# lean-dojo/ReProver

Hardware: NVIDIA H100
Metric: premises encoded/sec (reindex_corpus, ByT5-small, seq_len<=512) (higher is better)
Workload: dtype bf16

## Files before the change

reprover_b200/csrc/rpx_attention.cu:

```cuda
#include "rpx_common.cuh"
#include "rpx_kernels.cuh"
#include "rpx_ptx.cuh"

namespace rpx {

namespace {

constexpr int kHD = 64;
constexpr int kQT = 64;
constexpr int kKT = 64;
constexpr int kAttnThreads = 160;
constexpr int kTileBytes = 64 * 128;

constexpr int kOffQ = 0;
constexpr int kOffK = kTileBytes;
constexpr int kOffV = 3 * kTileBytes;
constexpr int kOffBias = 5 * kTileBytes;

__host__ __device__ constexpr int bias_floats(int R) { return ((2 * R + 1) + 3) & ~3; }
size_t attention_smem_bytes(int R) { return 1024 + kOffBias + (size_t)bias_floats(R) * 4 + 64; }

RPX_DEVICE float fast_exp2(float x) {
  float y;
  asm("ex2.approx.ftz.f32 %0, %1;" : "=f"(y) : "f"(x));
  return y;
}

__global__ void __launch_bounds__(kAttnThreads, 2)
t5_attention_kernel(const __grid_constant__ CUtensorMap tm_q, const __grid_constant__ CUtensorMap tm_kv,
                    __nv_bfloat16* __restrict__ out, const int32_t* __restrict__ cu_seqlens,
                    const float* __restrict__ bias_lut, int n_heads, int R, int ld_out) {
  const int seq = blockIdx.z, head = blockIdx.y, qt = blockIdx.x;
  pdl_launch_dependents();
  const int t0 = cu_seqlens[seq];
  const int len = cu_seqlens[seq + 1] - t0;
  const int q0 = qt * kQT;
  if (q0 >= len) return;

  extern __shared__ uint8_t smem_raw[];
  const uint32_t raw = smem_u32(smem_raw);
  uint8_t* smem = smem_raw + ((1024 - (raw & 1023)) & 1023);
  float* sBias = reinterpret_cast<float*>(smem + kOffBias);
  const int lut_w = 2 * R + 1;
  uint64_t* bars = reinterpret_cast<uint64_t*>(smem + kOffBias + bias_floats(R) * 4);
  uint64_t* bar_q = bars + 0;
  uint64_t* bar_k = bars + 1;
  uint64_t* bar_v = bars + 3;
  uint64_t* bar_free = bars + 5;

  const int warp = threadIdx.x >> 5, lane = threadIdx.x & 31;
  const int inner = n_heads * kHD;
  const int n_kt = (len + kKT - 1) / kKT;

  for (int i = threadIdx.x; i < lut_w; i += kAttnThreads) sBias[i] = bias_lut[head * lut_w + i];
  if (warp == 4) {
    if (elect_one()) {
      mbar_init(bar_q, 1);
      for (int b = 0; b < 2; ++b) {
        mbar_init(&bar_k[b], 1);
        mbar_init(&bar_v[b], 1);
        mbar_init(&bar_free[b], 128);
      }
      fence_mbar_init();
    }
    __syncwarp();
  }
  __syncthreads();

  if (warp == 4) {
    if (elect_one()) {
      const int kcol = inner + head * kHD, vcol = 2 * inner + head * kHD;
      pdl_wait();
      mbar_arrive_expect_tx(bar_q, kTileBytes);
      tma_load_2d(smem + kOffQ, &tm_q, bar_q, head * kHD, t0 + q0);
      for (int kt = 0; kt < n_kt; ++kt) {
        const int b = kt & 1;
        if (kt >= 2) mbar_wait<0>(&bar_free[b], ((kt >> 1) - 1) & 1);
        mbar_arrive_expect_tx(&bar_k[b], kTileBytes);
        tma_load_2d(smem + kOffK + b * kTileBytes, &tm_kv, &bar_k[b], kcol, t0 + kt * kKT);
        mbar_arrive_expect_tx(&bar_v[b], kTileBytes);
        tma_load_2d(smem + kOffV + b * kTileBytes, &tm_kv, &bar_v[b], vcol, t0 + kt * kKT);
      }
    }
  } else {
    const int g = lane >> 2, cq = 2 * (lane & 3);
    const int qpos0 = q0 + warp * 16 + g, qpos1 = qpos0 + 8;
    const float kLog2e = 1.4426950408889634f;
    float m0 = -INFINITY, m1 = -INFINITY, l0 = 0.f, l1 = 0.f;
    float o[32];
#pragma unroll
    for (int i = 0; i < 32; ++i) o[i] = 0.f;
    const uint64_t q_desc = make_smem_desc_kmajor_sw128(smem_u32(smem + kOffQ));
    mbar_wait<0>(bar_q, 0);
    for (int kt = 0; kt < n_kt; ++kt) {
      const int b = kt & 1;
      const uint32_t ph = (kt >> 1) & 1;
      const int kb = kt * kKT;
      float sc[32];
      mbar_wait<0>(&bar_k[b], ph);
      {
        const uint64_t k_desc = make_smem_desc_kmajor_sw128(smem_u32(smem + kOffK + b * kTileBytes));
        wgmma_fence_operand(sc);
        wgmma_fence();
#pragma unroll
        for (int k = 0; k < kHD / 16; ++k) wgmma_m64n64k16_ss(sc, q_desc + 2 * k, k_desc + 2 * k, k != 0);
        wgmma_commit();
        wgmma_wait<0>();
        wgmma_fence_operand(sc);
      }
      float mx0 = -INFINITY, mx1 = -INFINITY;
#pragma unroll
      for (int j = 0; j < 8; ++j) {
#pragma unroll
        for (int e = 0; e < 2; ++e) {
          const int key = kb + 8 * j + cq + e;
          const bool ok = key < len;
          const float b0 = sBias[min(max(key - qpos0 + R, 0), 2 * R)];
          const float b1 = sBias[min(max(key - qpos1 + R, 0), 2 * R)];
          sc[4 * j + e] = ok ? sc[4 * j + e] + b0 : -INFINITY;
          sc[4 * j + 2 + e] = ok ? sc[4 * j + 2 + e] + b1 : -INFINITY;
          mx0 = fmaxf(mx0, sc[4 * j + e]);
          mx1 = fmaxf(mx1, sc[4 * j + 2 + e]);
        }
      }
      mx0 = fmaxf(mx0, __shfl_xor_sync(0xffffffffu, mx0, 1));
      mx0 = fmaxf(mx0, __shfl_xor_sync(0xffffffffu, mx0, 2));
      mx1 = fmaxf(mx1, __shfl_xor_sync(0xffffffffu, mx1, 1));
      mx1 = fmaxf(mx1, __shfl_xor_sync(0xffffffffu, mx1, 2));
      const float mn0 = fmaxf(m0, mx0), mn1 = fmaxf(m1, mx1);
      const float scale0 = fast_exp2((m0 - mn0) * kLog2e), scale1 = fast_exp2((m1 - mn1) * kLog2e);
      m0 = mn0;
      m1 = mn1;
      const float mb0 = mn0 * kLog2e, mb1 = mn1 * kLog2e;
      uint32_t pa[4][4];
      float ls0 = 0.f, ls1 = 0.f;
#pragma unroll
      for (int j = 0; j < 8; ++j) {
        const float p00 = fast_exp2(fmaf(sc[4 * j], kLog2e, -mb0));
        const float p01 = fast_exp2(fmaf(sc[4 * j + 1], kLog2e, -mb0));
        const float p10 = fast_exp2(fmaf(sc[4 * j + 2], kLog2e, -mb1));
        const float p11 = fast_exp2(fmaf(sc[4 * j + 3], kLog2e, -mb1));
        ls0 += p00 + p01;
        ls1 += p10 + p11;
        pa[j >> 1][(j & 1) * 2] = pack_bf16x2(p00, p01);
        pa[j >> 1][(j & 1) * 2 + 1] = pack_bf16x2(p10, p11);
      }
      l0 = l0 * scale0 + ls0;
      l1 = l1 * scale1 + ls1;
#pragma unroll
      for (int j = 0; j < 8; ++j) {
        o[4 * j] *= scale0;
        o[4 * j + 1] *= scale0;
        o[4 * j + 2] *= scale1;
        o[4 * j + 3] *= scale1;
      }
      mbar_wait<0>(&bar_v[b], ph);
      {
        const uint32_t v_base = smem_u32(smem + kOffV + b * kTileBytes);
        wgmma_fence_operand(o);
        wgmma_fence();
#pragma unroll
        for (int c = 0; c < kKT / 16; ++c)
          wgmma_m64n64k16_rs_bmn(o, pa[c], make_smem_desc_mnmajor_sw128(v_base + c * 2048), 1);
        wgmma_commit();
        wgmma_wait<0>();
        wgmma_fence_operand(o);
      }
      mbar_arrive(&bar_free[b]);
    }
    l0 += __shfl_xor_sync(0xffffffffu, l0, 1);
    l0 += __shfl_xor_sync(0xffffffffu, l0, 2);
    l1 += __shfl_xor_sync(0xffffffffu, l1, 1);
    l1 += __shfl_xor_sync(0xffffffffu, l1, 2);
    const float inv0 = 1.f / l0, inv1 = 1.f / l1;
    __nv_bfloat16* dst0 = out + (int64_t)(t0 + qpos0) * ld_out + head * kHD + cq;
    __nv_bfloat16* dst1 = out + (int64_t)(t0 + qpos1) * ld_out + head * kHD + cq;
#pragma unroll
    for (int j = 0; j < 8; ++j) {
      if (qpos0 < len) *reinterpret_cast<uint32_t*>(dst0 + 8 * j) = pack_bf16x2(o[4 * j] * inv0, o[4 * j + 1] * inv0);
      if (qpos1 < len) *reinterpret_cast<uint32_t*>(dst1 + 8 * j) = pack_bf16x2(o[4 * j + 2] * inv1, o[4 * j + 3] * inv1);
    }
  }
}

}

int launch_t5_attention(const __nv_bfloat16* qkv, __nv_bfloat16* out, const int32_t* cu_seqlens,
                        const float* bias_lut, int n_tokens, int n_seqs, int max_len, int n_heads, int d_kv,
                        int max_distance, cudaStream_t stream) {
  RPX_REQUIRE(d_kv == kHD, RPX_ERR_UNSUPPORTED, "attention: d_kv=%d (only 64 is implemented)", d_kv);
  RPX_REQUIRE(n_seqs > 0 && max_len > 0 && n_tokens > 0, RPX_ERR_INVALID, "attention: empty batch");
  RPX_REQUIRE(n_seqs <= 65535 && n_heads <= 65535, RPX_ERR_UNSUPPORTED, "attention: grid limits exceeded");
  const int inner = n_heads * d_kv;
  DeviceInfo dev;
  RPX_TRY(get_device_info(&dev));
  CUtensorMap tm_q, tm_kv;
  RPX_TRY(make_tmap_bf16_2d(&tm_kv, qkv, (uint64_t)n_tokens, (uint64_t)3 * inner, (uint64_t)3 * inner, kKT));
  RPX_TRY(make_tmap_bf16_2d(&tm_q, qkv, (uint64_t)n_tokens, (uint64_t)3 * inner, (uint64_t)3 * inner, kQT));
  const size_t smem = attention_smem_bytes(max_distance);
  RPX_REQUIRE(smem <= 100 * 1024, RPX_ERR_UNSUPPORTED, "attention: bias table too large (%zu B of shared memory)", smem);
  static thread_local int configured = -1;
// ... 12 lines not shown
```

reprover_b200/csrc/rpx_encoder.cu:

```cuda
#include <math.h>

#include <new>
#include <vector>

#include "rpx_gemm_launch.cuh"
#include "rpx_kernels.cuh"

namespace rpx {

namespace {

constexpr int kBlockN = 128;

struct LayerW {
  const __nv_bfloat16* qkv;
  const __nv_bfloat16* o;
  const __nv_bfloat16* wi;
  const __nv_bfloat16* wo;
};

struct ProfRec {
  int cls;
  cudaEvent_t a, b;
};

}

}

extern "C" int32_t rpx_t5_relative_bucket(int32_t relative_position, int32_t num_buckets, int32_t max_distance) {
  int nb = num_buckets / 2;
  int ret = relative_position > 0 ? nb : 0;
  int n = relative_position < 0 ? -relative_position : relative_position;
  const int max_exact = nb / 2;
  if (n < max_exact) return ret + n;
  float v = logf((float)n / (float)max_exact) / (float)log((double)max_distance / (double)max_exact) *
            (float)(nb - max_exact);
  int large = max_exact + (int)v;
  if (large > nb - 1) large = nb - 1;
  return ret + large;
}

struct rpx_encoder {
  rpx_t5_config cfg;
  int inner = 0;
// ... 144 lines not shown
  }
  ~Prof() {
    if (!e->profiling) return;
    cudaEventRecord(b, st);
    e->prof_pending.push_back({cls, a, b});
  }
  cudaEvent_t get() {
    if (!e->event_pool.empty()) {
      cudaEvent_t ev = e->event_pool.back();
      e->event_pool.pop_back();
      return ev;
    }
    cudaEvent_t ev;
    cudaEventCreate(&ev);
    return ev;
  }
};

constexpr int kLatBlockN = 64;
constexpr int kLatStages = 6;
constexpr int kLatSmallM = 64;
constexpr int kLatSmallStages = 12;
constexpr int kLatSmallMMaxTokens = 384;
constexpr int kPdlMaxTokens = 16384;

struct PdlScope {
  explicit PdlScope(bool on) { set_pdl_scope(on); }
  ~PdlScope() { set_pdl_scope(false); }
};

int ss_parts(int d_model, bool latency) { return ceil_div(d_model, latency ? 32 : 128); }


int qkv_gemm(bool latency, int T, const void* A, const void* B, int N, int K, const RowScale& rs, __nv_bfloat16* out,
             const void* prefetch, size_t prefetch_bytes, cudaStream_t st) {
  EpiStoreBF16::Params ep{out, N, rs};
  if (!latency) return launch_gemm<kBlockN, EpiStoreBF16>(A, K, B, K, T, N, K, ep, st);
  if (T <= kLatSmallMMaxTokens)
    return launch_gemm<kLatBlockN, EpiStoreBF16, false, kLatSmallStages, false, kLatSmallM>(A, K, B, K, T, N, K, ep, st, 0,
                                                                                             prefetch, prefetch_bytes);
  return launch_gemm<kLatBlockN, EpiStoreBF16, false, kLatStages>(A, K, B, K, T, N, K, ep, st, 0, prefetch, prefetch_bytes);
}

template <int RES_BUFS, int STAGES, int CLUSTER>
int residual_gemm(bool latency, int T, const void* A, const void* B, int N, int K, float* h32, __nv_bfloat16* h16,
                  float* ss_out, cudaStream_t st) {
  EpiResidualParams ep{h32, h16, N, ss_out, T};
  if (!latency) return launch_gemm_ws<EpiWsResidual<RES_BUFS>, STAGES, CLUSTER>(A, K, B, K, T, N, K, ep, st);
  if (T <= kLatSmallMMaxTokens)
    return launch_gemm<kLatBlockN, EpiResidualChunkSS, false, kLatSmallStages, false, kLatSmallM>(A, K, B, K, T, N, K, ep, st);
  return launch_gemm<kLatBlockN, EpiResidualChunkSS, false, kLatStages>(A, K, B, K, T, N, K, ep, st);
}
int oproj_gemm(bool latency, int T, const void* A, const void* B, int N, int K, float* h32, __nv_bfloat16* h16,
               float* ss_out, cudaStream_t st) {
  return residual_gemm<2, 4, 1>(latency, T, A, B, N, K, h32, h16, ss_out, st);
}
int ffn_down_gemm(bool latency, int T, const void* A, const void* B, int N, int K, float* h32, __nv_bfloat16* h16,
                  float* ss_out, cudaStream_t st) {
  return residual_gemm<5, 3, 2>(latency, T, A, B, N, K, h32, h16, ss_out, st);
}

int ffn_up_gemm(bool latency, int T, const void* A, const void* B, int N, int K, const RowScale& rs,
                __nv_bfloat16* out, cudaStream_t st) {
  RPX_REQUIRE(N % 256 == 0, RPX_ERR_UNSUPPORTED, "ffn-up gemm: N=%d must be a multiple of 256 (2 x d_ff, d_ff %% 128 == 0)", N);
  const int F = N / 2;
  if (!latency) {
    EpiWsGeGLU::Params ep{out, F, rs};
    return launch_gemm_ws<EpiWsGeGLU, kFfnUpStages, kFfnUpCluster>(A, K, B, K, T, N, K, ep, st);
  }
  if (T <= kBlockM) {
// ... 405 lines not shown
```

reprover_b200/csrc/rpx_gemm_launch.cuh:

```cuda
#pragma once
#include "rpx_common.cuh"
#include "rpx_gemm.cuh"
#include "rpx_gemm_ws.cuh"

namespace rpx {

constexpr int kGemmStages = 4;

template <int BLOCK_N, class Epi, bool M_FASTEST = false, int STAGES = kGemmStages, bool SPLIT_B = false, int BM = kBlockM>
int launch_gemm(const void* A, int64_t lda, const void* B, int64_t ldb, int M, int N, int K,
                const typename Epi::Params& ep, cudaStream_t stream, int grid_limit = 0, const void* prefetch_ptr = nullptr,
                size_t prefetch_bytes = 0) {
  using Cfg = GemmCfg<BLOCK_N, STAGES, BM>;
  static_assert(BM == kBlockM || (!M_FASTEST && Epi::kWarps == 4), "64-row tiles: encoder epilogues with one warp per lane group");
  RPX_REQUIRE(M > 0 && N > 0 && K > 0, RPX_ERR_INVALID, "gemm: empty problem M=%d N=%d K=%d", M, N, K);
  RPX_REQUIRE(K % kBlockK == 0, RPX_ERR_UNSUPPORTED, "gemm: K=%d must be a multiple of %d", K, kBlockK);
  RPX_REQUIRE(M_FASTEST || N % 32 == 0, RPX_ERR_UNSUPPORTED, "gemm: N=%d must be a multiple of 32", N);
  DeviceInfo dev;
  RPX_TRY(get_device_info(&dev));
  CUtensorMap tmA, tmB;
  RPX_TRY(make_tmap_bf16_2d(&tmA, A, (uint64_t)M, (uint64_t)K, (uint64_t)lda, BM));
  RPX_TRY(make_tmap_bf16_2d(&tmB, B, (uint64_t)N, (uint64_t)K, (uint64_t)ldb, SPLIT_B ? BLOCK_N / 2 : BLOCK_N));
  RPX_REQUIRE(!SPLIT_B || N % BLOCK_N == 0, RPX_ERR_UNSUPPORTED, "gemm: split-B tiles need N %% %d == 0", BLOCK_N);
  const int tiles_m = ceil_div(M, BM);
  const int tiles_n = ceil_div(N, BLOCK_N);
  const size_t smem = Cfg::smem_bytes(Epi::kSmemBytes);
  RPX_REQUIRE(smem <= dev.smem_optin, RPX_ERR_UNSUPPORTED, "gemm: needs %zu B smem, device allows %zu",
              smem, dev.smem_optin);
  auto kern = gemm_tc_kernel<BLOCK_N, STAGES, Epi, M_FASTEST, SPLIT_B, BM>;
  static thread_local int configured_dev = -1;
  if (configured_dev != dev.device) {
    RPX_CUDA_OK(cudaFuncSetAttribute(kern, cudaFuncAttributeMaxDynamicSharedMemorySize, (int)smem));
    configured_dev = dev.device;
  }
  int grid = tiles_m * tiles_n;
  int cap = grid_limit > 0 ? grid_limit : dev.num_sms;
  if (grid > cap) grid = cap;
  L2Prefetch pf{prefetch_ptr, (uint32_t)prefetch_bytes, grid, next_timeline_slot()};
  if (prefetch_ptr != nullptr && prefetch_bytes > 0 && prefetch_bytes < ((size_t)1 << 32) && grid < dev.num_sms)
    grid = dev.num_sms;
  RPX_CUDA_OK(launch_pdl(kern, dim3(grid), dim3(gemm_threads<Epi>()), smem, stream, pdl_enabled(), tmA, tmB, M, N, K, tiles_m,
                         tiles_n, 1, ep, pf));
  return RPX_OK;
}

constexpr int kFfnUpStages = 4;
constexpr int kFfnUpCluster = 2;

template <class Epi, int STAGES, int CLUSTER>
int launch_gemm_ws(const void* A, int64_t lda, const void* B, int64_t ldb, int M, int N, int K,
                   const typename Epi::Params& ep, cudaStream_t stream) {
  RPX_REQUIRE(M > 0 && N > 0 && K > 0, RPX_ERR_INVALID, "gemm: empty problem M=%d N=%d K=%d", M, N, K);
  RPX_REQUIRE(K % kBlockK == 0, RPX_ERR_UNSUPPORTED, "gemm: K=%d must be a multiple of %d", K, kBlockK);
  RPX_REQUIRE(N % 32 == 0, RPX_ERR_UNSUPPORTED, "gemm: N=%d must be a multiple of 32", N);
  DeviceInfo dev;
  RPX_TRY(get_device_info(&dev));
  CUtensorMap tmA, tmB, tmR;
  RPX_TRY(make_tmap_bf16_2d(&tmA, A, (uint64_t)M, (uint64_t)K, (uint64_t)lda, kBlockM));
  RPX_TRY(make_tmap_bf16_2d(&tmB, B, (uint64_t)N, (uint64_t)K, (uint64_t)ldb, kWsBlockN / CLUSTER));
  if constexpr (Epi::kResBufs > 0)
    RPX_TRY(make_tmap_2d(&tmR, 4, ep.h32, (uint64_t)M, (uint64_t)N, (uint64_t)ep.ld, kResChunkCols, 64, 128));
  else
    tmR = tmA;
  const int tiles_m = ceil_div(M, kBlockM);
  const int tiles_n = ceil_div(N, kWsBlockN);
  const size_t smem = WsCfg<STAGES, Epi::kResBufs>::kSmemBytes;
  RPX_REQUIRE(smem <= dev.smem_optin, RPX_ERR_UNSUPPORTED, "gemm: needs %zu B smem, device allows %zu", smem,
              dev.smem_optin);
  auto kern = gemm_ws_kernel<Epi, STAGES, CLUSTER>;
  static thread_local int configured_dev = -1;
  static thread_local int max_clusters = 0;
  if (configured_dev != dev.device) {
    RPX_CUDA_OK(cudaFuncSetAttribute(kern, cudaFuncAttributeMaxDynamicSharedMemorySize, (int)smem));
    cudaLaunchConfig_t cfg{};
    cfg.gridDim = dim3(CLUSTER * dev.num_sms);
    cfg.blockDim = dim3(kWsThreads);
    cfg.dynamicSmemBytes = smem;
    cudaLaunchAttribute at[1];
    at[0].id = cudaLaunchAttributeClusterDimension;
    at[0].val.clusterDim.x = CLUSTER;
    at[0].val.clusterDim.y = 1;
    at[0].val.clusterDim.z = 1;
    cfg.attrs = at;
    cfg.numAttrs = 1;
    RPX_CUDA_OK(cudaOccupancyMaxActiveClusters(&max_clusters, kern, &cfg));
    RPX_REQUIRE(max_clusters > 0, RPX_ERR_UNSUPPORTED, "gemm: no cluster of %d CTAs with %zu B smem fits the device",
                CLUSTER, smem);
    configured_dev = dev.device;
  }
  int clusters = ceil_div(tiles_m, CLUSTER) * tiles_n;
  if (clusters > max_clusters) clusters = max_clusters;
  RPX_CUDA_OK(launch_pdl<CLUSTER>(kern, dim3(CLUSTER * clusters), dim3(kWsThreads), smem, stream, pdl_enabled(), tmA,
                                  tmB, tmR, M, N, K, tiles_m, tiles_n, ep));
  return RPX_OK;
}

template <class Epi, int STAGES = kGemmStages>
int launch_gemm_pair(const void* A, int64_t lda, const void* B, int64_t ldb, int M, int N, int K,
                     const typename Epi::Params& ep, cudaStream_t stream) {
  constexpr int BLOCK_N = 128;
  using Cfg = GemmCfg<BLOCK_N, STAGES, kBlockM>;
  RPX_REQUIRE(M > 0 && N > 0 && K > 0, RPX_ERR_INVALID, "gemm: empty problem M=%d N=%d K=%d", M, N, K);
// ... 39 lines not shown
```

reprover_b200/csrc/rpx_gemm_ws.cuh:

```cuda
#pragma once
#include "rpx_gemm.cuh"

namespace rpx {

constexpr int kWsBlockN = 256;
constexpr int kWsThreads = 384;
constexpr int kResChunkCols = 32;
constexpr int kResChunkBytes = 64 * kResChunkCols * 4;

template <int STAGES, int RES_BUFS>
struct WsCfg {
  static_assert(2 * STAGES + 4 * RES_BUFS <= 32, "barrier block holds 32 mbarriers");
  static constexpr int kABytes = kBlockM * kBlockK * 2;
  static constexpr int kBBytes = kWsBlockN * kBlockK * 2;
  static constexpr int kStageBytes = kABytes + kBBytes;
  static constexpr int kRingBytes = STAGES * kStageBytes;
  static constexpr int kResBytes = 2 * RES_BUFS * kResChunkBytes;
  static constexpr size_t kSmemBytes = (size_t)kRingBytes + kResBytes + 1024 + 256;
};

struct FragCtx {
  int m0, n0;
  int n_blk;
  int n_cols;
  int M, N;
  int r0;
  int q;
};

struct ResStream {
  float* buf;
  uint64_t* full;
  uint64_t* empty;
};

template <class Epi, int STAGES, int CLUSTER>
__global__ void __launch_bounds__(kWsThreads, 1)
gemm_ws_kernel(const __grid_constant__ CUtensorMap tmA, const __grid_constant__ CUtensorMap tmB,
               const __grid_constant__ CUtensorMap tmR, int M, int N, int K, int tiles_m, int tiles_n,
               typename Epi::Params ep) {
  static_assert(CLUSTER == 1 || CLUSTER == 2, "one CTA, or a pair sharing the B tile");
  using Cfg = WsCfg<STAGES, Epi::kResBufs>;
  constexpr int R = Epi::kResBufs;
  extern __shared__ uint8_t smem_raw[];
  const uint32_t raw_addr = smem_u32(smem_raw);
  uint8_t* smem = smem_raw + ((1024 - (raw_addr & 1023)) & 1023);
  uint8_t* sA = smem;
  uint8_t* sB = smem + STAGES * Cfg::kABytes;
  float* sR = reinterpret_cast<float*>(smem + Cfg::kRingBytes);
  uint64_t* full = reinterpret_cast<uint64_t*>(smem + Cfg::kRingBytes + Cfg::kResBytes);
  uint64_t* empty = full + STAGES;
  uint64_t* rfull = empty + STAGES;
  uint64_t* rempty = rfull + 2 * R;

  const int warp = threadIdx.x >> 5;
  const int wg = warp >> 2;
  const int num_kb = K / kBlockK;
  const int rank = CLUSTER > 1 ? (int)cluster_ctarank() : 0;
  const int num_units = (tiles_m + CLUSTER - 1) / CLUSTER * tiles_n;
  const int u0 = (int)blockIdx.x / CLUSTER;
  const int u_step = (int)gridDim.x / CLUSTER;
  auto unit_m = [&](int u) { return CLUSTER * (u / tiles_n) + rank; };

  if (threadIdx.x == 0) {
    tma_prefetch_desc(&tmA);
    tma_prefetch_desc(&tmB);
    if (R > 0) tma_prefetch_desc(&tmR);
    for (int s = 0; s < STAGES; ++s) {
      mbar_init(&full[s], 1);
      mbar_init(&empty[s], CLUSTER * 8);
    }
    for (int s = 0; s < 2 * R; ++s) {
      mbar_init(&rfull[s], 1);
      mbar_init(&rempty[s], 128);
    }
    fence_mbar_init();
  }
  __syncthreads();
  if (CLUSTER > 1) cluster_sync_all();
  pdl_launch_dependents();
  pdl_wait();

  if (wg == 0) {
    setmaxnreg_dec<40>();
    if (warp == 0 && elect_one()) {
      int stage = 0;
      uint32_t phase = 0;
      for (int u = u0; u < num_units; u += u_step) {
        const int m_blk = unit_m(u), n_blk = u % tiles_n;
        for (int kb = 0; kb < num_kb; ++kb) {
          mbar_wait(&empty[stage], phase ^ 1);
          mbar_arrive_expect_tx(&full[stage], Cfg::kStageBytes);
          tma_load_2d(sA + stage * Cfg::kABytes, &tmA, &full[stage], kb * kBlockK, m_blk * kBlockM);
          if constexpr (CLUSTER == 1) {
            tma_load_2d(sB + stage * Cfg::kBBytes, &tmB, &full[stage], kb * kBlockK, n_blk * kWsBlockN);
          } else {
            constexpr int H = kWsBlockN / 2;
            tma_load_2d_multicast(sB + stage * Cfg::kBBytes + rank * H * kBlockK * 2, &tmB, &full[stage], kb * kBlockK,
                                  n_blk * kWsBlockN + rank * H, (uint16_t)0x3);
          }
          if (++stage == STAGES) {
            stage = 0;
            phase ^= 1;
          }
        }
      }
    } else if (R > 0 && (warp == 1 || warp == 2) && elect_one()) {
      const int w = warp - 1;
      float* buf = sR + w * R * (kResChunkBytes / 4);
      uint64_t* rf = rfull + w * R;
      uint64_t* re = rempty + w * R;
      int b = 0;
      uint32_t phase = 0;
      for (int u = u0; u < num_units; u += u_step) {
        const int row0 = unit_m(u) * kBlockM + 64 * w;
        const int n0 = (u % tiles_n) * kWsBlockN;
        const int n_cols = N - n0 < kWsBlockN ? N - n0 : kWsBlockN;
        if (row0 >= M) continue;
        for (int col = 0; col < n_cols; col += kResChunkCols) {
          mbar_wait(&re[b], phase ^ 1);
          mbar_arrive_expect_tx(&rf[b], kResChunkBytes);
          tma_load_2d(buf + b * (kResChunkBytes / 4), &tmR, &rf[b], n0 + col, row0);
          if (++b == R) {
            b = 0;
            phase ^= 1;
          }
        }
      }
    }
  } else {
    setmaxnreg_inc<232>();
    const int cw = wg - 1;
    const int lane = threadIdx.x & 31;
    Epi epi(ep, ResStream{sR + cw * R * (kResChunkBytes / 4), rfull + cw * R, rempty + cw * R});
    float acc[128];
    int stage = 0;
    uint32_t phase = 0;
    auto release = [&](int st) {
      __syncwarp();
      if (lane == 0) {
        mbar_arrive(&empty[st]);
        if (CLUSTER > 1) mbar_arrive_cluster(&empty[st], (uint32_t)(rank ^ 1));
      }
    };
    for (int u = u0; u < num_units; u += u_step) {
      FragCtx c;
      c.n_blk = u % tiles_n;
      c.m0 = unit_m(u) * kBlockM;
      c.n0 = c.n_blk * kWsBlockN;
      c.n_cols = N - c.n0 < kWsBlockN ? N - c.n0 : kWsBlockN;
      c.M = M;
      c.N = N;
      c.r0 = c.m0 + 64 * cw + 16 * (warp & 3) + (lane >> 2);
      c.q = lane & 3;
      int prev = 0;
      for (int kb = 0; kb < num_kb; ++kb) {
        mbar_wait(&full[stage], phase);
        const uint64_t a_desc = make_smem_desc_kmajor_sw128(smem_u32(sA + stage * Cfg::kABytes)) + 512 * cw;
        const uint64_t b_desc = make_smem_desc_kmajor_sw128(smem_u32(sB + stage * Cfg::kBBytes));
        wgmma_fence_operand(acc);
        wgmma_fence();
#pragma unroll
        for (int k = 0; k < kBlockK / kMmaK; ++k) wgmma_m64n256k16_ss(acc, a_desc + 2 * k, b_desc + 2 * k, (kb | k) != 0);
        wgmma_commit();
        if (kb == 0) epi.prefetch(c);
        if (kb > 0) {
          wgmma_wait<1>();
          release(prev);
        }
        prev = stage;
        if (++stage == STAGES) {
          stage = 0;
          phase ^= 1;
        }
      }
      wgmma_wait<0>();
      wgmma_fence_operand(acc);
      release(prev);
      epi.tile(c, acc);
    }
  }
  if (CLUSTER > 1) {
    __syncwarp();
    cluster_sync_all();
  }
}


struct EpiWsStoreF32 {
  using Params = EpiStoreF32::Params;
  static constexpr int kResBufs = 0;
  Params p;
  __device__ EpiWsStoreF32(const Params& p_, const ResStream&) : p(p_) {}
  __device__ void prefetch(const FragCtx&) {}
  __device__ void tile(const FragCtx& c, const float (&acc)[128]) {
#pragma unroll
    for (int j = 0; j < 32; ++j) {
      if (8 * j < c.n_cols) {
        float* dst = p.C + (size_t)c.r0 * p.ldc + c.n0 + 8 * j + 2 * c.q;
        if (c.r0 < c.M) *reinterpret_cast<float2*>(dst) = make_float2(acc[4 * j], acc[4 * j + 1]);
        if (c.r0 + 8 < c.M) *reinterpret_cast<float2*>(dst + 8 * (size_t)p.ldc) = make_float2(acc[4 * j + 2], acc[4 * j + 3]);
      }
    }
  }
};

struct EpiWsGeGLU {
  struct Params {
    __nv_bfloat16* out;
    int ldo;
    RowScale rs;
  };
  static constexpr int kResBufs = 0;
  Params p;
  float rs0 = 0.f, rs1 = 0.f;
  __device__ EpiWsGeGLU(const Params& p_, const ResStream&) : p(p_) {}
  __device__ void prefetch(const FragCtx& c) {
    rs0 = c.r0 < c.M ? p.rs.get(c.r0) : 0.f;
    rs1 = c.r0 + 8 < c.M ? p.rs.get(c.r0 + 8) : 0.f;
  }
// ... 93 lines not shown
```

reprover_b200/csrc/rpx_ptx.cuh:

```cuda
#pragma once
#include <cuda_runtime.h>
#include <cuda_bf16.h>
#include <stdint.h>

namespace rpx {

#define RPX_DEVICE __device__ __forceinline__

RPX_DEVICE uint32_t smem_u32(const void* p) {
  return static_cast<uint32_t>(__cvta_generic_to_shared(p));
}

RPX_DEVICE uint32_t lane_id() { return threadIdx.x & 31; }

RPX_DEVICE uint32_t elect_one() {
  uint32_t pred = 0;
  asm volatile(
      "{\n"
      ".reg .b32 rx;\n"
      ".reg .pred px;\n"
      "elect.sync rx|px, 0xFFFFFFFF;\n"
      "@px mov.s32 %0, 1;\n"
      "}\n"
      : "+r"(pred));
// ... 135 lines not shown
RPX_DEVICE void wgmma_wait() {
  asm volatile("wgmma.wait_group.sync.aligned %0;" ::"n"(N) : "memory");
}
template <int R>
RPX_DEVICE void wgmma_fence_operand(float (&d)[R]) {
#pragma unroll
  for (int i = 0; i < R; ++i) asm volatile("" : "+f"(d[i])::"memory");
}

RPX_DEVICE void wgmma_m64n64k16_ss(float (&d)[32], uint64_t desc_a, uint64_t desc_b, uint32_t accumulate) {
  asm volatile(
      "{\n"
      ".reg .pred p;\n"
      "setp.ne.b32 p, %34, 0;\n"
      "wgmma.mma_async.sync.aligned.m64n64k16.f32.bf16.bf16 "
      "{%0, %1, %2, %3, %4, %5, %6, %7, %8, %9, %10, %11, %12, %13, %14, %15, %16, %17, %18, %19, %20, %21, %22, %23, %24, %25, %26, %27, %28, %29, %30, %31}, %32, %33, p, 1, 1, 0, 0;\n"
      "}\n"
      : "+f"(d[0]), "+f"(d[1]), "+f"(d[2]), "+f"(d[3]), "+f"(d[4]), "+f"(d[5]), "+f"(d[6]), "+f"(d[7]), "+f"(d[8]), "+f"(d[9]), "+f"(d[10]), "+f"(d[11]), "+f"(d[12]), "+f"(d[13]), "+f"(d[14]), "+f"(d[15]), "+f"(d[16]), "+f"(d[17]), "+f"(d[18]), "+f"(d[19]), "+f"(d[20]), "+f"(d[21]), "+f"(d[22]), "+f"(d[23]), "+f"(d[24]), "+f"(d[25]), "+f"(d[26]), "+f"(d[27]), "+f"(d[28]), "+f"(d[29]), "+f"(d[30]), "+f"(d[31])
      : "l"(desc_a), "l"(desc_b), "r"(accumulate));
}

RPX_DEVICE void wgmma_m64n128k16_ss(float (&d)[64], uint64_t desc_a, uint64_t desc_b, uint32_t accumulate) {
  asm volatile(
      "{\n"
      ".reg .pred p;\n"
      "setp.ne.b32 p, %66, 0;\n"
      "wgmma.mma_async.sync.aligned.m64n128k16.f32.bf16.bf16 "
      "{%0, %1, %2, %3, %4, %5, %6, %7, %8, %9, %10, %11, %12, %13, %14, %15, %16, %17, %18, %19, %20, %21, %22, %23, %24, %25, %26, %27, %28, %29, %30, %31, %32, %33, %34, %35, %36, %37, %38, %39, %40, %41, %42, %43, %44, %45, %46, %47, %48, %49, %50, %51, %52, %53, %54, %55, %56, %57, %58, %59, %60, %61, %62, %63}, %64, %65, p, 1, 1, 0, 0;\n"
      "}\n"
      : "+f"(d[0]), "+f"(d[1]), "+f"(d[2]), "+f"(d[3]), "+f"(d[4]), "+f"(d[5]), "+f"(d[6]), "+f"(d[7]), "+f"(d[8]), "+f"(d[9]), "+f"(d[10]), "+f"(d[11]), "+f"(d[12]), "+f"(d[13]), "+f"(d[14]), "+f"(d[15]), "+f"(d[16]), "+f"(d[17]), "+f"(d[18]), "+f"(d[19]), "+f"(d[20]), "+f"(d[21]), "+f"(d[22]), "+f"(d[23]), "+f"(d[24]), "+f"(d[25]), "+f"(d[26]), "+f"(d[27]), "+f"(d[28]), "+f"(d[29]), "+f"(d[30]), "+f"(d[31]), "+f"(d[32]), "+f"(d[33]), "+f"(d[34]), "+f"(d[35]), "+f"(d[36]), "+f"(d[37]), "+f"(d[38]), "+f"(d[39]), "+f"(d[40]), "+f"(d[41]), "+f"(d[42]), "+f"(d[43]), "+f"(d[44]), "+f"(d[45]), "+f"(d[46]), "+f"(d[47]), "+f"(d[48]), "+f"(d[49]), "+f"(d[50]), "+f"(d[51]), "+f"(d[52]), "+f"(d[53]), "+f"(d[54]), "+f"(d[55]), "+f"(d[56]), "+f"(d[57]), "+f"(d[58]), "+f"(d[59]), "+f"(d[60]), "+f"(d[61]), "+f"(d[62]), "+f"(d[63])
      : "l"(desc_a), "l"(desc_b), "r"(accumulate));
}

RPX_DEVICE void wgmma_m64n256k16_ss(float (&d)[128], uint64_t desc_a, uint64_t desc_b, uint32_t accumulate) {
  asm volatile(
      "{\n"
      ".reg .pred p;\n"
      "setp.ne.b32 p, %130, 0;\n"
      "wgmma.mma_async.sync.aligned.m64n256k16.f32.bf16.bf16 "
      "{%0, %1, %2, %3, %4, %5, %6, %7, %8, %9, %10, %11, %12, %13, %14, %15, %16, %17, %18, %19, %20, %21, %22, %23, %24, %25, %26, %27, %28, %29, %30, %31, %32, %33, %34, %35, %36, %37, %38, %39, %40, %41, %42, %43, %44, %45, %46, %47, %48, %49, %50, %51, %52, %53, %54, %55, %56, %57, %58, %59, %60, %61, %62, %63, %64, %65, %66, %67, %68, %69, %70, %71, %72, %73, %74, %75, %76, %77, %78, %79, %80, %81, %82, %83, %84, %85, %86, %87, %88, %89, %90, %91, %92, %93, %94, %95, %96, %97, %98, %99, %100, %101, %102, %103, %104, %105, %106, %107, %108, %109, %110, %111, %112, %113, %114, %115, %116, %117, %118, %119, %120, %121, %122, %123, %124, %125, %126, %127}, %128, %129, p, 1, 1, 0, 0;\n"
      "}\n"
      : "+f"(d[0]), "+f"(d[1]), "+f"(d[2]), "+f"(d[3]), "+f"(d[4]), "+f"(d[5]), "+f"(d[6]), "+f"(d[7]), "+f"(d[8]), "+f"(d[9]), "+f"(d[10]), "+f"(d[11]), "+f"(d[12]), "+f"(d[13]), "+f"(d[14]), "+f"(d[15]), "+f"(d[16]), "+f"(d[17]), "+f"(d[18]), "+f"(d[19]), "+f"(d[20]), "+f"(d[21]), "+f"(d[22]), "+f"(d[23]), "+f"(d[24]), "+f"(d[25]), "+f"(d[26]), "+f"(d[27]), "+f"(d[28]), "+f"(d[29]), "+f"(d[30]), "+f"(d[31]), "+f"(d[32]), "+f"(d[33]), "+f"(d[34]), "+f"(d[35]), "+f"(d[36]), "+f"(d[37]), "+f"(d[38]), "+f"(d[39]), "+f"(d[40]), "+f"(d[41]), "+f"(d[42]), "+f"(d[43]), "+f"(d[44]), "+f"(d[45]), "+f"(d[46]), "+f"(d[47]), "+f"(d[48]), "+f"(d[49]), "+f"(d[50]), "+f"(d[51]), "+f"(d[52]), "+f"(d[53]), "+f"(d[54]), "+f"(d[55]), "+f"(d[56]), "+f"(d[57]), "+f"(d[58]), "+f"(d[59]), "+f"(d[60]), "+f"(d[61]), "+f"(d[62]), "+f"(d[63]), "+f"(d[64]), "+f"(d[65]), "+f"(d[66]), "+f"(d[67]), "+f"(d[68]), "+f"(d[69]), "+f"(d[70]), "+f"(d[71]), "+f"(d[72]), "+f"(d[73]), "+f"(d[74]), "+f"(d[75]), "+f"(d[76]), "+f"(d[77]), "+f"(d[78]), "+f"(d[79]), "+f"(d[80]), "+f"(d[81]), "+f"(d[82]), "+f"(d[83]), "+f"(d[84]), "+f"(d[85]), "+f"(d[86]), "+f"(d[87]), "+f"(d[88]), "+f"(d[89]), "+f"(d[90]), "+f"(d[91]), "+f"(d[92]), "+f"(d[93]), "+f"(d[94]), "+f"(d[95]), "+f"(d[96]), "+f"(d[97]), "+f"(d[98]), "+f"(d[99]), "+f"(d[100]), "+f"(d[101]), "+f"(d[102]), "+f"(d[103]), "+f"(d[104]), "+f"(d[105]), "+f"(d[106]), "+f"(d[107]), "+f"(d[108]), "+f"(d[109]), "+f"(d[110]), "+f"(d[111]), "+f"(d[112]), "+f"(d[113]), "+f"(d[114]), "+f"(d[115]), "+f"(d[116]), "+f"(d[117]), "+f"(d[118]), "+f"(d[119]), "+f"(d[120]), "+f"(d[121]), "+f"(d[122]), "+f"(d[123]), "+f"(d[124]), "+f"(d[125]), "+f"(d[126]), "+f"(d[127])
      : "l"(desc_a), "l"(desc_b), "r"(accumulate));
}

RPX_DEVICE void wgmma_m64n64k16_rs_bmn(float (&d)[32], const uint32_t (&a)[4], uint64_t desc_b, uint32_t accumulate) {
  asm volatile(
      "{\n"
      ".reg .pred p;\n"
      "setp.ne.b32 p, %37, 0;\n"
      "wgmma.mma_async.sync.aligned.m64n64k16.f32.bf16.bf16 "
      "{%0, %1, %2, %3, %4, %5, %6, %7, %8, %9, %10, %11, %12, %13, %14, %15, %16, %17, %18, %19, %20, %21, %22, %23, %24, %25, %26, %27, %28, %29, %30, %31}, {%32, %33, %34, %35}, %36, p, 1, 1, 1;\n"
      "}\n"
      : "+f"(d[0]), "+f"(d[1]), "+f"(d[2]), "+f"(d[3]), "+f"(d[4]), "+f"(d[5]), "+f"(d[6]), "+f"(d[7]), "+f"(d[8]), "+f"(d[9]), "+f"(d[10]), "+f"(d[11]), "+f"(d[12]), "+f"(d[13]), "+f"(d[14]), "+f"(d[15]), "+f"(d[16]), "+f"(d[17]), "+f"(d[18]), "+f"(d[19]), "+f"(d[20]), "+f"(d[21]), "+f"(d[22]), "+f"(d[23]), "+f"(d[24]), "+f"(d[25]), "+f"(d[26]), "+f"(d[27]), "+f"(d[28]), "+f"(d[29]), "+f"(d[30]), "+f"(d[31])
      : "r"(a[0]), "r"(a[1]), "r"(a[2]), "r"(a[3]), "l"(desc_b), "r"(accumulate));
}

RPX_DEVICE uint64_t make_smem_desc_sw128(uint32_t smem_addr, uint32_t lbo_bytes) {
  uint64_t d = 0;
  d |= static_cast<uint64_t>((smem_addr & 0x3FFFF) >> 4);
  d |= static_cast<uint64_t>(lbo_bytes >> 4) << 16;
  d |= static_cast<uint64_t>(1024 >> 4) << 32;
  d |= static_cast<uint64_t>(1) << 62;
  return d;
}
RPX_DEVICE uint64_t make_smem_desc_kmajor_sw128(uint32_t smem_addr) { return make_smem_desc_sw128(smem_addr, 16); }
// ... 17 lines not shown
```

Baseline: 4309.

## Drop attention producer warp, specialize bias paths, route QKV GEMM to warp-specialized BN=192

The attention kernel removes its dedicated TMA producer warp and the free-barriers. Thread 0 now issues the K/V loads after a block-wide sync each iteration, so the block shrinks to 128 threads with a target of 5 CTAs per SM. Relative-position bias addition gains fast paths for tiles that are fully clamped or fully inside the bias window, masking runs only on the tail tile, and the O rescale is skipped when the scale is 1. Separately, the throughput QKV projection moves to the warp-specialized GEMM with a new 192-wide N tile via m64n192k16 wgmma and a new bf16 store epilogue. Risks include the per-iteration __syncthreads, which serializes loads behind compute, and register pressure under the tighter launch bound.

```diff
diff --git a/reprover_b200/csrc/rpx_attention.cu b/reprover_b200/csrc/rpx_attention.cu
--- a/reprover_b200/csrc/rpx_attention.cu
+++ b/reprover_b200/csrc/rpx_attention.cu
@@ -9,7 +9,8 @@
 constexpr int kHD = 64;
 constexpr int kQT = 64;
 constexpr int kKT = 64;
-constexpr int kAttnThreads = 160;
+constexpr int kAttnThreads = 128;
+constexpr int kAttnCtasPerSm = 5;
 constexpr int kTileBytes = 64 * 128;
 
 constexpr int kOffQ = 0;
@@ -26,7 +27,7 @@
   return y;
 }
 
-__global__ void __launch_bounds__(kAttnThreads, 2)
+__global__ void __launch_bounds__(kAttnThreads, kAttnCtasPerSm)
 t5_attention_kernel(const __grid_constant__ CUtensorMap tm_q, const __grid_constant__ CUtensorMap tm_kv,
                     __nv_bfloat16* __restrict__ out, const int32_t* __restrict__ cu_seqlens,
                     const float* __restrict__ bias_lut, int n_heads, int R, int ld_out) {
@@ -46,43 +47,36 @@
   uint64_t* bar_q = bars + 0;
   uint64_t* bar_k = bars + 1;
   uint64_t* bar_v = bars + 3;
-  uint64_t* bar_free = bars + 5;
 
   const int warp = threadIdx.x >> 5, lane = threadIdx.x & 31;
   const int inner = n_heads * kHD;
   const int n_kt = (len + kKT - 1) / kKT;
 
   for (int i = threadIdx.x; i < lut_w; i += kAttnThreads) sBias[i] = bias_lut[head * lut_w + i];
-  if (warp == 4) {
-    if (elect_one()) {
-      mbar_init(bar_q, 1);
-      for (int b = 0; b < 2; ++b) {
-        mbar_init(&bar_k[b], 1);
-        mbar_init(&bar_v[b], 1);
-        mbar_init(&bar_free[b], 128);
-      }
-      fence_mbar_init();
+  const int kcol = inner + head * kHD, vcol = 2 * inner + head * kHD;
+  auto load_kv = [&](int kt) {
+    const int b = kt & 1;
+    mbar_arrive_expect_tx(&bar_k[b], kTileBytes);
+    tma_load_2d(smem + kOffK + b * kTileBytes, &tm_kv, &bar_k[b], kcol, t0 + kt * kKT);
+    mbar_arrive_expect_tx(&bar_v[b], kTileBytes);
+    tma_load_2d(smem + kOffV + b * kTileBytes, &tm_kv, &bar_v[b], vcol, t0 + kt * kKT);
+  };
+  if (threadIdx.x == 0) {
+    mbar_init(bar_q, 1);
+    for (int b = 0; b < 2; ++b) {
+      mbar_init(&bar_k[b], 1);
+      mbar_init(&bar_v[b], 1);
     }
-    __syncwarp();
+    fence_mbar_init();
+    pdl_wait();
+    mbar_arrive_expect_tx(bar_q, kTileBytes);
+    tma_load_2d(smem + kOffQ, &tm_q, bar_q, head * kHD, t0 + q0);
+    load_kv(0);
+    if (n_kt > 1) load_kv(1);
   }
   __syncthreads();
 
-  if (warp == 4) {
-    if (elect_one()) {
-      const int kcol = inner + head * kHD, vcol = 2 * inner + head * kHD;
-      pdl_wait();
-      mbar_arrive_expect_tx(bar_q, kTileBytes);
-      tma_load_2d(smem + kOffQ, &tm_q, bar_q, head * kHD, t0 + q0);
-      for (int kt = 0; kt < n_kt; ++kt) {
-        const int b = kt & 1;
-        if (kt >= 2) mbar_wait<0>(&bar_free[b], ((kt >> 1) - 1) & 1);
-        mbar_arrive_expect_tx(&bar_k[b], kTileBytes);
-        tma_load_2d(smem + kOffK + b * kTileBytes, &tm_kv, &bar_k[b], kcol, t0 + kt * kKT);
-        mbar_arrive_expect_tx(&bar_v[b], kTileBytes);
-        tma_load_2d(smem + kOffV + b * kTileBytes, &tm_kv, &bar_v[b], vcol, t0 + kt * kKT);
-      }
-    }
-  } else {
+  {
     const int g = lane >> 2, cq = 2 * (lane & 3);
     const int qpos0 = q0 + warp * 16 + g, qpos1 = qpos0 + 8;
     const float kLog2e = 1.4426950408889634f;
@@ -92,33 +86,69 @@
     for (int i = 0; i < 32; ++i) o[i] = 0.f;
     const uint64_t q_desc = make_smem_desc_kmajor_sw128(smem_u32(smem + kOffQ));
     mbar_wait<0>(bar_q, 0);
-    for (int kt = 0; kt < n_kt; ++kt) {
+    auto issue_qk = [&](float (&sc)[32], int kt) {
       const int b = kt & 1;
-      const uint32_t ph = (kt >> 1) & 1;
+      mbar_wait<0>(&bar_k[b], (kt >> 1) & 1);
+      const uint64_t k_desc = make_smem_desc_kmajor_sw128(smem_u32(smem + kOffK + b * kTileBytes));
+      wgmma_fence_operand(sc);
+      wgmma_fence();
+#pragma unroll
+      for (int k = 0; k < kHD / 16; ++k) wgmma_m64n64k16_ss(sc, q_desc + 2 * k, k_desc + 2 * k, k != 0);
+      wgmma_commit();
+    };
+    auto softmax_issue_pv = [&](const float (&acc)[32], int kt) {
+      const int b = kt & 1;
       const int kb = kt * kKT;
+      const int d_lo = kb - q0 - (kQT - 1), d_hi = kb + (kKT - 1) - q0;
       float sc[32];
-      mbar_wait<0>(&bar_k[b], ph);
-      {
-        const uint64_t k_desc = make_smem_desc_kmajor_sw128(smem_u32(smem + kOffK + b * kTileBytes));
-        wgmma_fence_operand(sc);
-        wgmma_fence();
-#pragma unroll
-        for (int k = 0; k < kHD / 16; ++k) wgmma_m64n64k16_ss(sc, q_desc + 2 * k, k_desc + 2 * k, k != 0);
-        wgmma_commit();
-        wgmma_wait<0>();
-        wgmma_fence_operand(sc);
+      if (d_hi <= -R || d_lo >= R) {
+        const float bc = sBias[d_hi <= -R ? 0 : 2 * R];
+#pragma unroll
+        for (int i = 0; i < 32; ++i) sc[i] = acc[i] + bc;
+      } else if (d_lo >= -R && d_hi <= R) {
+        const float* bp = sBias + (kb + cq - qpos0 + R - 8);
+        float t[9][2];
+#pragma unroll
+        for (int i = 0; i < 9; ++i) {
+          t[i][0] = bp[8 * i];
+          t[i][1] = bp[8 * i + 1];
+        }
+#pragma unroll
+        for (int j = 0; j < 8; ++j) {
+#pragma unroll
+          for (int e = 0; e < 2; ++e) {
+            sc[4 * j + e] = acc[4 * j + e] + t[j + 1][e];
+            sc[4 * j + 2 + e] = acc[4 * j + 2 + e] + t[j][e];
+          }
+        }
+      } else {
+#pragma unroll
+        for (int j = 0; j < 8; ++j) {
+#pragma unroll
+          for (int e = 0; e < 2; ++e) {
+            const int key = kb + 8 * j + cq + e;
+            sc[4 * j + e] = acc[4 * j + e] + sBias[min(max(key - qpos0 + R, 0), 2 * R)];
+            sc[4 * j + 2 + e] = acc[4 * j + 2 + e] + sBias[min(max(key - qpos1 + R, 0), 2 * R)];
+          }
+        }
+      }
+      if (kb + kKT > len) {
+#pragma unroll
+        for (int j = 0; j < 8; ++j) {
+#pragma unroll
+          for (int e = 0; e < 2; ++e) {
+            if (kb + 8 * j + cq + e >= len) {
+              sc[4 * j + e] = -INFINITY;
+              sc[4 * j + 2 + e] = -INFINITY;
+            }
+          }
+        }
       }
       float mx0 = -INFINITY, mx1 = -INFINITY;
 #pragma unroll
       for (int j = 0; j < 8; ++j) {
 #pragma unroll
         for (int e = 0; e < 2; ++e) {
-          const int key = kb + 8 * j + cq + e;
-          const bool ok = key < len;
-          const float b0 = sBias[min(max(key - qpos0 + R, 0), 2 * R)];
-          const float b1 = sBias[min(max(key - qpos1 + R, 0), 2 * R)];
-          sc[4 * j + e] = ok ? sc[4 * j + e] + b0 : -INFINITY;
-          sc[4 * j + 2 + e] = ok ? sc[4 * j + 2 + e] + b1 : -INFINITY;
           mx0 = fmaxf(mx0, sc[4 * j + e]);
           mx1 = fmaxf(mx1, sc[4 * j + 2 + e]);
         }
@@ -147,26 +177,41 @@
       }
       l0 = l0 * scale0 + ls0;
       l1 = l1 * scale1 + ls1;
-#pragma unroll
-      for (int j = 0; j < 8; ++j) {
-        o[4 * j] *= scale0;
-        o[4 * j + 1] *= scale0;
-        o[4 * j + 2] *= scale1;
-        o[4 * j + 3] *= scale1;
-      }
-      mbar_wait<0>(&bar_v[b], ph);
-      {
-        const uint32_t v_base = smem_u32(smem + kOffV + b * kTileBytes);
-        wgmma_fence_operand(o);
-        wgmma_fence();
-#pragma unroll
-        for (int c = 0; c < kKT / 16; ++c)
-          wgmma_m64n64k16_rs_bmn(o, pa[c], make_smem_desc_mnmajor_sw128(v_base + c * 2048), 1);
-        wgmma_commit();
-        wgmma_wait<0>();
-        wgmma_fence_operand(o);
-      }
-      mbar_arrive(&bar_free[b]);
+      if (scale0 != 1.f) {
+#pragma unroll
+        for (int j = 0; j < 8; ++j) {
+          o[4 * j] *= scale0;
+          o[4 * j + 1] *= scale0;
+        }
+      }
+      if (scale1 != 1.f) {
+#pragma unroll
+        for (int j = 0; j < 8; ++j) {
+          o[4 * j + 2] *= scale1;
+          o[4 * j + 3] *= scale1;
+        }
+      }
+      mbar_wait<0>(&bar_v[b], (kt >> 1) & 1);
+      const uint32_t v_base = smem_u32(smem + kOffV + b * kTileBytes);
+      wgmma_fence_operand(o);
+      wgmma_fence();
+#pragma unroll
+      for (int c = 0; c < kKT / 16; ++c)
+        wgmma_m64n64k16_rs_bmn(o, pa[c], make_smem_desc_mnmajor_sw128(v_base + c * 2048), 1);
+      wgmma_commit();
+    };
+    float sa[32];
+    for (int kt = 0; kt < n_kt; ++kt) {
+      issue_qk(sa, kt);
+      wgmma_wait<0>();
+      wgmma_fence_operand(sa);
+      softmax_issue_pv(sa, kt);
+      wgmma_wait<0>();
+      wgmma_fence_operand(o);
+      if (kt + 2 < n_kt) {
+        __syncthreads();
+        if (threadIdx.x == 0) load_kv(kt + 2);
+      }
     }
     l0 += __shfl_xor_sync(0xffffffffu, l0, 1);
     l0 += __shfl_xor_sync(0xffffffffu, l0, 2);
diff --git a/reprover_b200/csrc/rpx_encoder.cu b/reprover_b200/csrc/rpx_encoder.cu
--- a/reprover_b200/csrc/rpx_encoder.cu
+++ b/reprover_b200/csrc/rpx_encoder.cu
@@ -9,8 +9,6 @@
 namespace rpx {
 
 namespace {
-
-constexpr int kBlockN = 128;
 
 struct LayerW {
   const __nv_bfloat16* qkv;
@@ -221,10 +219,12 @@
 int ss_parts(int d_model, bool latency) { return ceil_div(d_model, latency ? 32 : 128); }
 
 
+constexpr int kQkvStages = 4;
+constexpr int kQkvCluster = 1;
 int qkv_gemm(bool latency, int T, const void* A, const void* B, int N, int K, const RowScale& rs, __nv_bfloat16* out,
              const void* prefetch, size_t prefetch_bytes, cudaStream_t st) {
   EpiStoreBF16::Params ep{out, N, rs};
-  if (!latency) return launch_gemm<kBlockN, EpiStoreBF16>(A, K, B, K, T, N, K, ep, st);
+  if (!latency) return launch_gemm_ws<EpiWsStoreBF16, kQkvStages, kQkvCluster, 192>(A, K, B, K, T, N, K, ep, st);
   if (T <= kLatSmallMMaxTokens)
     return launch_gemm<kLatBlockN, EpiStoreBF16, false, kLatSmallStages, false, kLatSmallM>(A, K, B, K, T, N, K, ep, st, 0,
                                                                                              prefetch, prefetch_bytes);
diff --git a/reprover_b200/csrc/rpx_gemm_launch.cuh b/reprover_b200/csrc/rpx_gemm_launch.cuh
--- a/reprover_b200/csrc/rpx_gemm_launch.cuh
+++ b/reprover_b200/csrc/rpx_gemm_launch.cuh
@@ -47,7 +47,7 @@
 constexpr int kFfnUpStages = 4;
 constexpr int kFfnUpCluster = 2;
 
-template <class Epi, int STAGES, int CLUSTER>
+template <class Epi, int STAGES, int CLUSTER, int BN = kWsBlockN>
 int launch_gemm_ws(const void* A, int64_t lda, const void* B, int64_t ldb, int M, int N, int K,
                    const typename Epi::Params& ep, cudaStream_t stream) {
   RPX_REQUIRE(M > 0 && N > 0 && K > 0, RPX_ERR_INVALID, "gemm: empty problem M=%d N=%d K=%d", M, N, K);
@@ -57,17 +57,17 @@
   RPX_TRY(get_device_info(&dev));
   CUtensorMap tmA, tmB, tmR;
   RPX_TRY(make_tmap_bf16_2d(&tmA, A, (uint64_t)M, (uint64_t)K, (uint64_t)lda, kBlockM));
-  RPX_TRY(make_tmap_bf16_2d(&tmB, B, (uint64_t)N, (uint64_t)K, (uint64_t)ldb, kWsBlockN / CLUSTER));
+  RPX_TRY(make_tmap_bf16_2d(&tmB, B, (uint64_t)N, (uint64_t)K, (uint64_t)ldb, BN / CLUSTER));
   if constexpr (Epi::kResBufs > 0)
     RPX_TRY(make_tmap_2d(&tmR, 4, ep.h32, (uint64_t)M, (uint64_t)N, (uint64_t)ep.ld, kResChunkCols, 64, 128));
   else
     tmR = tmA;
   const int tiles_m = ceil_div(M, kBlockM);
-  const int tiles_n = ceil_div(N, kWsBlockN);
-  const size_t smem = WsCfg<STAGES, Epi::kResBufs>::kSmemBytes;
+  const int tiles_n = ceil_div(N, BN);
+  const size_t smem = WsCfg<STAGES, Epi::kResBufs, BN>::kSmemBytes;
   RPX_REQUIRE(smem <= dev.smem_optin, RPX_ERR_UNSUPPORTED, "gemm: needs %zu B smem, device allows %zu", smem,
               dev.smem_optin);
-  auto kern = gemm_ws_kernel<Epi, STAGES, CLUSTER>;
+  auto kern = gemm_ws_kernel<Epi, STAGES, CLUSTER, BN>;
   static thread_local int configured_dev = -1;
   static thread_local int max_clusters = 0;
   if (configured_dev != dev.device) {
diff --git a/reprover_b200/csrc/rpx_gemm_ws.cuh b/reprover_b200/csrc/rpx_gemm_ws.cuh
--- a/reprover_b200/csrc/rpx_gemm_ws.cuh
+++ b/reprover_b200/csrc/rpx_gemm_ws.cuh
@@ -8,11 +8,12 @@
 constexpr int kResChunkCols = 32;
 constexpr int kResChunkBytes = 64 * kResChunkCols * 4;
 
-template <int STAGES, int RES_BUFS>
+template <int STAGES, int RES_BUFS, int BN>
 struct WsCfg {
   static_assert(2 * STAGES + 4 * RES_BUFS <= 32, "barrier block holds 32 mbarriers");
+  static_assert(BN == 256 || BN == 192, "wgmma.m64n256k16 or m64n192k16 per consumer");
   static constexpr int kABytes = kBlockM * kBlockK * 2;
-  static constexpr int kBBytes = kWsBlockN * kBlockK * 2;
+  static constexpr int kBBytes = BN * kBlockK * 2;
   static constexpr int kStageBytes = kABytes + kBBytes;
   static constexpr int kRingBytes = STAGES * kStageBytes;
   static constexpr int kResBytes = 2 * RES_BUFS * kResChunkBytes;
@@ -34,13 +35,13 @@
   uint64_t* empty;
 };
 
-template <class Epi, int STAGES, int CLUSTER>
+template <class Epi, int STAGES, int CLUSTER, int BN>
 __global__ void __launch_bounds__(kWsThreads, 1)
 gemm_ws_kernel(const __grid_constant__ CUtensorMap tmA, const __grid_constant__ CUtensorMap tmB,
                const __grid_constant__ CUtensorMap tmR, int M, int N, int K, int tiles_m, int tiles_n,
                typename Epi::Params ep) {
   static_assert(CLUSTER == 1 || CLUSTER == 2, "one CTA, or a pair sharing the B tile");
-  using Cfg = WsCfg<STAGES, Epi::kResBufs>;
+  using Cfg = WsCfg<STAGES, Epi::kResBufs, BN>;
   constexpr int R = Epi::kResBufs;
   extern __shared__ uint8_t smem_raw[];
   const uint32_t raw_addr = smem_u32(smem_raw);
@@ -93,11 +94,11 @@
           mbar_arrive_expect_tx(&full[stage], Cfg::kStageBytes);
           tma_load_2d(sA + stage * Cfg::kABytes, &tmA, &full[stage], kb * kBlockK, m_blk * kBlockM);
           if constexpr (CLUSTER == 1) {
-            tma_load_2d(sB + stage * Cfg::kBBytes, &tmB, &full[stage], kb * kBlockK, n_blk * kWsBlockN);
+            tma_load_2d(sB + stage * Cfg::kBBytes, &tmB, &full[stage], kb * kBlockK, n_blk * BN);
           } else {
-            constexpr int H = kWsBlockN / 2;
+            constexpr int H = BN / 2;
             tma_load_2d_multicast(sB + stage * Cfg::kBBytes + rank * H * kBlockK * 2, &tmB, &full[stage], kb * kBlockK,
-                                  n_blk * kWsBlockN + rank * H, (uint16_t)0x3);
+                                  n_blk * BN + rank * H, (uint16_t)0x3);
           }
           if (++stage == STAGES) {
             stage = 0;
@@ -114,8 +115,8 @@
       uint32_t phase = 0;
       for (int u = u0; u < num_units; u += u_step) {
         const int row0 = unit_m(u) * kBlockM + 64 * w;
-        const int n0 = (u % tiles_n) * kWsBlockN;
-        const int n_cols = N - n0 < kWsBlockN ? N - n0 : kWsBlockN;
+        const int n0 = (u % tiles_n) * BN;
+        const int n_cols = N - n0 < BN ? N - n0 : BN;
         if (row0 >= M) continue;
         for (int col = 0; col < n_cols; col += kResChunkCols) {
           mbar_wait(&re[b], phase ^ 1);
@@ -133,7 +134,7 @@
     const int cw = wg - 1;
     const int lane = threadIdx.x & 31;
     Epi epi(ep, ResStream{sR + cw * R * (kResChunkBytes / 4), rfull + cw * R, rempty + cw * R});
-    float acc[128];
+    float acc[BN / 2];
     int stage = 0;
     uint32_t phase = 0;
     auto release = [&](int st) {
@@ -147,8 +148,8 @@
       FragCtx c;
       c.n_blk = u % tiles_n;
       c.m0 = unit_m(u) * kBlockM;
-      c.n0 = c.n_blk * kWsBlockN;
-      c.n_cols = N - c.n0 < kWsBlockN ? N - c.n0 : kWsBlockN;
+      c.n0 = c.n_blk * BN;
+      c.n_cols = N - c.n0 < BN ? N - c.n0 : BN;
       c.M = M;
       c.N = N;
       c.r0 = c.m0 + 64 * cw + 16 * (warp & 3) + (lane >> 2);
@@ -161,7 +162,12 @@
         wgmma_fence_operand(acc);
         wgmma_fence();
 #pragma unroll
-        for (int k = 0; k < kBlockK / kMmaK; ++k) wgmma_m64n256k16_ss(acc, a_desc + 2 * k, b_desc + 2 * k, (kb | k) != 0);
+        for (int k = 0; k < kBlockK / kMmaK; ++k) {
+          if constexpr (BN == 256)
+            wgmma_m64n256k16_ss(acc, a_desc + 2 * k, b_desc + 2 * k, (kb | k) != 0);
+          else
+            wgmma_m64n192k16_ss(acc, a_desc + 2 * k, b_desc + 2 * k, (kb | k) != 0);
+        }
         wgmma_commit();
         if (kb == 0) epi.prefetch(c);
         if (kb > 0) {
@@ -186,6 +192,30 @@
   }
 }
 
+
+struct EpiWsStoreBF16 {
+  using Params = EpiStoreBF16::Params;
+  static constexpr int kResBufs = 0;
+  Params p;
+  float rs0 = 0.f, rs1 = 0.f;
+  __device__ EpiWsStoreBF16(const Params& p_, const ResStream&) : p(p_) {}
+  __device__ void prefetch(const FragCtx& c) {
+    rs0 = c.r0 < c.M ? p.rs.get(c.r0) : 0.f;
+    rs1 = c.r0 + 8 < c.M ? p.rs.get(c.r0 + 8) : 0.f;
+  }
+  template <int R>
+  __device__ void tile(const FragCtx& c, const float (&acc)[R]) {
+    __nv_bfloat16* dst = p.C + (size_t)c.r0 * p.ldc + c.n0 + 2 * c.q;
+#pragma unroll
+    for (int j = 0; j < R / 4; ++j) {
+      if (8 * j < c.n_cols) {
+        if (c.r0 < c.M) *reinterpret_cast<uint32_t*>(dst + 8 * j) = pack_bf16x2(acc[4 * j] * rs0, acc[4 * j + 1] * rs0);
+        if (c.r0 + 8 < c.M)
+          *reinterpret_cast<uint32_t*>(dst + 8 * (size_t)p.ldc + 8 * j) = pack_bf16x2(acc[4 * j + 2] * rs1, acc[4 * j + 3] * rs1);
+      }
+    }
+  }
+};
 
 struct EpiWsStoreF32 {
   using Params = EpiStoreF32::Params;
diff --git a/reprover_b200/csrc/rpx_ptx.cuh b/reprover_b200/csrc/rpx_ptx.cuh
--- a/reprover_b200/csrc/rpx_ptx.cuh
+++ b/reprover_b200/csrc/rpx_ptx.cuh
@@ -191,6 +191,18 @@
       : "l"(desc_a), "l"(desc_b), "r"(accumulate));
 }
 
+RPX_DEVICE void wgmma_m64n192k16_ss(float (&d)[96], uint64_t desc_a, uint64_t desc_b, uint32_t accumulate) {
+  asm volatile(
+      "{\n"
+      ".reg .pred p;\n"
+      "setp.ne.b32 p, %98, 0;\n"
+      "wgmma.mma_async.sync.aligned.m64n192k16.f32.bf16.bf16 "
+      "{%0, %1, %2, %3, %4, %5, %6, %7, %8, %9, %10, %11, %12, %13, %14, %15, %16, %17, %18, %19, %20, %21, %22, %23, %24, %25, %26, %27, %28, %29, %30, %31, %32, %33, %34, %35, %36, %37, %38, %39, %40, %41, %42, %43, %44, %45, %46, %47, %48, %49, %50, %51, %52, %53, %54, %55, %56, %57, %58, %59, %60, %61, %62, %63, %64, %65, %66, %67, %68, %69, %70, %71, %72, %73, %74, %75, %76, %77, %78, %79, %80, %81, %82, %83, %84, %85, %86, %87, %88, %89, %90, %91, %92, %93, %94, %95}, %96, %97, p, 1, 1, 0, 0;\n"
+      "}\n"
+      : "+f"(d[0]), "+f"(d[1]), "+f"(d[2]), "+f"(d[3]), "+f"(d[4]), "+f"(d[5]), "+f"(d[6]), "+f"(d[7]), "+f"(d[8]), "+f"(d[9]), "+f"(d[10]), "+f"(d[11]), "+f"(d[12]), "+f"(d[13]), "+f"(d[14]), "+f"(d[15]), "+f"(d[16]), "+f"(d[17]), "+f"(d[18]), "+f"(d[19]), "+f"(d[20]), "+f"(d[21]), "+f"(d[22]), "+f"(d[23]), "+f"(d[24]), "+f"(d[25]), "+f"(d[26]), "+f"(d[27]), "+f"(d[28]), "+f"(d[29]), "+f"(d[30]), "+f"(d[31]), "+f"(d[32]), "+f"(d[33]), "+f"(d[34]), "+f"(d[35]), "+f"(d[36]), "+f"(d[37]), "+f"(d[38]), "+f"(d[39]), "+f"(d[40]), "+f"(d[41]), "+f"(d[42]), "+f"(d[43]), "+f"(d[44]), "+f"(d[45]), "+f"(d[46]), "+f"(d[47]), "+f"(d[48]), "+f"(d[49]), "+f"(d[50]), "+f"(d[51]), "+f"(d[52]), "+f"(d[53]), "+f"(d[54]), "+f"(d[55]), "+f"(d[56]), "+f"(d[57]), "+f"(d[58]), "+f"(d[59]), "+f"(d[60]), "+f"(d[61]), "+f"(d[62]), "+f"(d[63]), "+f"(d[64]), "+f"(d[65]), "+f"(d[66]), "+f"(d[67]), "+f"(d[68]), "+f"(d[69]), "+f"(d[70]), "+f"(d[71]), "+f"(d[72]), "+f"(d[73]), "+f"(d[74]), "+f"(d[75]), "+f"(d[76]), "+f"(d[77]), "+f"(d[78]), "+f"(d[79]), "+f"(d[80]), "+f"(d[81]), "+f"(d[82]), "+f"(d[83]), "+f"(d[84]), "+f"(d[85]), "+f"(d[86]), "+f"(d[87]), "+f"(d[88]), "+f"(d[89]), "+f"(d[90]), "+f"(d[91]), "+f"(d[92]), "+f"(d[93]), "+f"(d[94]), "+f"(d[95])
+      : "l"(desc_a), "l"(desc_b), "r"(accumulate));
+}
+
 RPX_DEVICE void wgmma_m64n256k16_ss(float (&d)[128], uint64_t desc_a, uint64_t desc_b, uint32_t accumulate) {
   asm volatile(
       "{\n"
```

Measured after the change: 4385 (median of 6 runs). 1.8% higher.
